# FlowEternal/multitask-hydranet

Measured on AMD Instinct MI355X. Metric: images/sec (fwd+bwd) HydraNet @ default res, 1/2/4/8 MI355X; CPU-ref same run, higher is better.
Workload: dtype bf16; 1 GPU; full HydraNet (backbone + BiFPN + seg/det/lane heads + multitask loss), big cfg, fwd+loss+bwd; batch_per_gpu=16, global_batch=16, resolution=3x512x1024, parallelism=dp1, hipgraph=True

## Files before the change

include/hydranet_hip.h:

```cpp
#ifndef HYDRANET_HIP_H
#define HYDRANET_HIP_H

#ifdef __cplusplus
extern "C" {
#endif

typedef struct ihipStream_t* hipStream_t;


int hn_gconv_pack_diag(const float* w, void* wk, void* wd, int C, hipStream_t stream);
int hn_pack_weight(const float* w, void* wp, void* wt, int Cout, int Cin, int taps, hipStream_t stream);
int hn_pack_weight_ex(const float* w, void* wp, void* wt, int Cout, int Cin_total, int ci0, int Cin, int taps, int phase, const float* bias,
                      float* b_eff, hipStream_t stream);
int hn_phase_fold(const float* dw_eff, const float* dw1, const float* db_eff, float* dw, float* db, int K, int C0, int C1, hipStream_t stream);
int hn_pack_weights_batched(const long* jobs, int njobs, long total_blocks, const int* block_job, hipStream_t stream);
int hn_pack_small_batched(const long* jobs, const int* block_job, long total_blocks, hipStream_t stream);

int hn_conv_gemm_nt(const void* x0, const void* x1, int mode, int n_img, int H, int W, int C0, int C1, int ld0, int ld1, int up, long M,
                    const void* w, int Nout, int KP, int taps, const float* bias, int act, void* out, int out_f32, int ldc, long rpi,
                    long img_stride, float* psum, float* psq, hipStream_t stream);
int hn_nt_stat_rows(long M, int Nout);
int hn_nt_stat_tile(long M, int Nout);
int hn_direct_stat_rows(int n_img, int H, int W);
int hn_conv_gemm_nt_imgw(const void* x0, int ld0, long M, int C0, const void* w, long w_img_stride, long rows_per_image, int Nout, int KP,
                         const float* bias, int act, void* out, int ldc, const void* addend, int ld_add, hipStream_t stream);
int hn_scale_weight_gate(const void* wp, const float* gate, void* out, int N, int Cout, int C, int KP, hipStream_t stream);
int hn_conv_gemm_nt_lvl(const void* x0, int ld0, long M, int C0, const void* w, int Nout, int KP, const float* bias, int act, void* out,
                        int ldc, const float* coef, int nlev, const long* rows, hipStream_t stream);
int hn_conv_gemm_nt_lvlout(const void* x0, int ld0, long M, int C0, const void* w, int Nout, int KP, const float* bias, int act, float* out,
                           int ldc, long img_stride, int n_img, int nlev, const int* H, const int* W, int row_align, hipStream_t stream);

int hn_conv_gemm_nt_ex(const void* x0, const void* x1, int mode, int n_img, int H, int W, int C0, int C1, int ld0, int ld1, int up, long M,
                       const void* w, int Nout, int KP, int taps, const float* bias, int act, void* out, int out_f32, int ldc, long rpi,
                       long img_stride, float* psum, float* psq, const float* xscale, const float* xshift, const float* xgate, long xhw,
                       int xact, const void* addend, int ld_add, int add_mode, hipStream_t stream);
int hn_conv_gemm_nt_stat(const void* x0, const void* x1, int mode, int n_img, int H, int W, int C0, int C1, int ld0, int ld1, int up, long M,
                         const void* w, int Nout, int KP, int taps, const float* bias, int act, void* out, int out_f32, int ldc, long rpi,
                         long img_stride, float* psum, float* psq, const void* addend, int ld_add, int add_mode, int emode, const void* ez,
                         int ld_ez, const float* ecoef, hipStream_t stream);
int hn_conv_gemm_nt_stat3(const void* x0, int ld0, long M, int C0, const void* w, int Nout, int KP, void* out, int ldc, float* psum, float* psq,
                          const void* addend, int ld_add, const void* ez, int ld_ez, const void* ey, int ld_ey, const float* ecoef,
                          hipStream_t stream);
int hn_wgrad_plan(int mode, int n_img, int H, int W, long M, int Nout, int KP, int taps, int* splits, long* rows_per_split, long* ws_bytes);
int hn_conv_gemm_tn(const void* x0, const void* x1, int mode, int n_img, int H, int W, int C0, int C1, int ld0, int ld1, int up, long M,
                    const void* dz, int ldz, int Nout, int KP, int taps, float* workspace, float* dw, hipStream_t stream);


int hn_stem_fwd(const float* x, const float* w, void* z, void* patches, int N, int H, int W, hipStream_t stream);

int hn_gconv_pack(const float* w, void* wk, void* wd, int C, int flip, hipStream_t stream);
int hn_gconv_fwd(const void* in, int ldi, const void* wk, void* out, int ldo, int N, int Hi, int Wi, int C, int stride, hipStream_t stream);
int hn_gconv_dgrad_s2(const void* dz, int ldz, const void* wd, void* dx, int ldx, int N, int Hi, int Wi, int C, hipStream_t stream);
long hn_wgrad_chunks(long pixels, long items);
int hn_gconv_wgrad(const void* x, int ldx, const void* dz, int ldz, float* part, int N, int Hi, int Wi, int C, int stride,
                   hipStream_t stream);

int hn_dw_pack(const float* w, void* wk, void* wkf, int C, hipStream_t stream);
int hn_dwconv_fwd(const void* in, int ldi, const void* wk, void* out, int ldo, int N, int H, int W, int C, hipStream_t stream);
int hn_dwconv_fwd_levels(const void* in, int ldi, const void* wk, void* out, int ldo, int N, int C, int nlev, const int* H, const int* W,
                         int row_align, int accumulate, hipStream_t stream);
long hn_dwconv_wgrad_blocks(long strips, int C);
int hn_dwconv_wgrad(const void* x, int ldx, const void* dz, int ldz, float* part, int N, int H, int W, int C, hipStream_t stream);
int hn_dwconv_wgrad_levels(const void* x, int ldx, const void* dz, int ldz, float* part, int N, int C, int nlev, const int* H, const int* W,
                           int row_align, hipStream_t stream);
long hn_dwconv_bwd_blocks(long strips, int C);
long hn_dwconv_bwd_blocks_levels(int N, int C, int nlev, const int* H, const int* W);
int hn_dwconv_bwd_levels(const void* dz, int ldz, const void* x, int ldx, const void* wf, void* dx, int lddx, float* part, int N, int C,
                         int nlev, const int* H, const int* W, int row_align, int accumulate, hipStream_t stream);

int hn_maxpool_fwd(const void* in, int ldi, void* out, int ldo, int N, int H, int W, int C, int mode, hipStream_t stream);
int hn_maxpool_bwd(const void* in, int ldi, const void* dout, int ldd, void* dx, int ldx, const float* wscale, int N, int H, int W, int C,
                   int mode, hipStream_t stream);
int hn_maxpool_bwd2(const void* in, int ldi, const void* dout, int ldd, void* dx, int ldx, const float* wscale, void* arg_ws, int N, int H,
                    int W, int C, int mode, int accumulate, hipStream_t stream);

int hn_up2_fwd(const void* in, int ldi, void* out, int ldo, int N, int H, int W, int C, hipStream_t stream);
int hn_sum2x2(const void* g, int ldg, void* out, int ldo, const float* wscale, int N, int H, int W, int C, int accumulate, hipStream_t stream);

int hn_fuse_dweights(const float* pw, int blocks, const float* praw, int nw, float eps, float* dp, hipStream_t stream);
int hn_fuse_fwd(const void* const* in, const int* ld, const int* mode, const float* w, void* out, int ldo, int N, int H, int W, int C,
                hipStream_t stream);
int hn_fuse_fwd_raw(const void* const* in, const int* ld, const int* mode, const float* praw, int nw, float eps, float* wn, void* out, int ldo,
                    int N, int H, int W, int C, hipStream_t stream);
int hn_fuse_bwd_blocks(int N, int H, int W, int C);
int hn_fuse_bwd(const void* const* in, const int* ld, const int* mode, const float* w, const void* dout, int ldd, void* g, int ldg,
                void* const* din, const int* ldin, const int* acc, float* pw, int N, int H, int W, int C, hipStream_t stream);
int hn_fuse_bwd_arg(const void* const* in, const int* ld, const int* mode, const float* w, const void* dout, int ldd, void* g, int ldg,
                    void* const* din, const int* ldin, const int* acc, float* pw, void* const* arg_out, int N, int H, int W, int C,
                    hipStream_t stream);
int hn_maxpool_bwd_from_arg(const void* arg, const void* dout, int ldd, void* dx, int ldx, const float* wscale, int N, int H, int W, int C,
                            int mode, int accumulate, hipStream_t stream);

// ... 206 lines not shown
```

multitask_hydranet_amd/csrc/hn_gemm.hip:

```cpp
#include "hn_common.h"
#include <climits>

#ifdef HN_TUNING
#define HN_DBG(p) ((p).dbg)
#else
#define HN_DBG(p) 0
#endif

struct XSrc {
    const bf16* x0;
    const bf16* x1;
    int mode;
    int H, W;
    int Hi, Wi;
    int C0, C1;
    int ld0, ld1;
    int up;
    long M;
    int clamp;
    int diag;
};

__device__ __forceinline__ int border_idx(int v, int L, int clamp) {
    if (clamp == 2) return (v < 0 || v >= L) ? -1 : v;
// ... 60 lines not shown
    if (s.mode == 2) {
        int iy = oy + ky - 1, ix = ox + kx - 1;
        iy = iy < 0 ? -iy : (iy >= s.Hi ? 2 * s.Hi - 2 - iy : iy);
        ix = ix < 0 ? -ix : (ix >= s.Wi ? 2 * s.Wi - 2 - ix : ix);
        if (which) return s.C1 ? (((long)n * s.Hi + iy) * s.Wi + ix) * s.ld1 : -1;
        const int hh = s.Hi >> s.up, ww = s.Wi >> s.up;
        return (((long)n * hh + (iy >> s.up)) * ww + (ix >> s.up)) * s.ld0;
    }
    const int iy = oy - ky, ix = ox - kx;
    if (which || iy < 0 || iy >= s.Hi || ix < 0 || ix >= s.Wi) return -1;
    return (((long)n * s.Hi + iy) * s.Wi + ix) * s.ld0;
}

__device__ __forceinline__ void glds16(const bf16* src, char* lds_wave_base) {
    __builtin_amdgcn_global_load_lds((const __attribute__((address_space(1))) void*)src,
                                     (__attribute__((address_space(3))) void*)lds_wave_base, 16, 0, 0);
}

__device__ __forceinline__ int swz(int row, int piece) { return row * 128 + ((piece ^ (row & 7)) << 4); }
__device__ __forceinline__ int pswz32(int row) { return (row >> 1) & 2; }

struct GemmNT {
    XSrc x;
    const bf16* w;
    int Nout, KP, taps;
    const float* bias;
    int act;
    void* out;
    int ldc;
    float* psum;
    float* psq;
    long rpi;
    long img_stride;
    int d2s;
    const float* xscale; const float* xshift; const float* xgate; long xhw; int xact;
    const bf16* addend; int ld_add;
    int phase_mode, phase_span;
    int add_s2;
    long* amax;
    int add_pre;
    long w_img_stride; unsigned w_rpi;
    const float* lcoef; int ln; long lrow[HN_MAX_LEVELS + 1];
    int lo_n; unsigned lo_hw[HN_MAX_LEVELS]; unsigned lo_pix[HN_MAX_LEVELS];
    int fold;
    bf16* fold_out2; int ld_fo2;
    bf16* ring;
    const bf16* fold_y; int ld_fy;
    int emode; const bf16* ez; int ld_ez; const float* ecoef;
    const bf16* ey; int ld_ey;
    int tile_major;
    int wpre;
    unsigned long long* dbg_buf;
    int dbg;
};

struct StatCoef { f32x4 sc, sh, mu, rs; };
__device__ __forceinline__ StatCoef stat_coef(const float* ecoef, int Nout, int emode, int co0, bool ev) {
    StatCoef c;
    c.sc = c.sh = c.mu = c.rs = (f32x4){0.f, 0.f, 0.f, 0.f};
    if (ev) {
        c.sc = *reinterpret_cast<const f32x4*>(ecoef + co0);
        c.sh = *reinterpret_cast<const f32x4*>(ecoef + Nout + co0);
        if (emode == 2) {
            c.mu = *reinterpret_cast<const f32x4*>(ecoef + 2 * Nout + co0);
            c.rs = *reinterpret_cast<const f32x4*>(ecoef + 3 * Nout + co0);
        }
    }
    return c;
}
__device__ __forceinline__ void stat_terms4(int emode, const f32x4 q, const f32x4 z, const StatCoef& cf, float& a0, float& a1, float& a2, float& a3,
                                            float& b0, float& b1, float& b2, float& b3) {
    float t1[4], t2[4];
#pragma unroll
    for (int r = 0; r < 4; ++r) {
        const float pre = cf.sc[r] * z[r] + cf.sh[r];
        const float b = bfround(pre > 0.f ? pre : 0.f);
        const float g = pre > 0.f ? q[r] : 0.f;
        t1[r] = emode == 0 ? q[r] : (emode == 1 ? q[r] * b : g);
        t2[r] = emode == 0 ? q[r] * q[r] : g * (z[r] - cf.mu[r]) * cf.rs[r];
    }
    a0 += t1[0]; a1 += t1[1]; a2 += t1[2]; a3 += t1[3];
    b0 += t2[0]; b1 += t2[1]; b2 += t2[2]; b3 += t2[3];
}

template <int BC, int BP, int WGC, int WGP, bool OUT_F32, int R, bool XF = false, int KG = 1, bool PLAIN = false, bool EPRE = false>
__global__ __launch_bounds__(256 * KG) void gemm_nt_kernel(const GemmNT p) {
    static_assert(!XF || R == 2, "the register-staged operand transform is written for the double buffer");
    static_assert(!PLAIN || !XF, "the plain-rows form has no operand transform");
    static_assert(KG == 1 || (!XF && R == 2), "the K-group form is written for the plain double buffer");
    constexpr int WC = BC / WGC, WP = BP / WGP, TC = WC / 16, TP = WP / 16;
    constexpr int XR = BP / 32, WR = (BC + 31) / 32;
    constexpr int STAGE = (BC + BP) * 128;
    extern __shared__ __attribute__((aligned(16))) char smem[];
    const int tid = threadIdx.x & 255, kg = __builtin_amdgcn_readfirstlane(threadIdx.x >> 8), lane = tid & 63, wave = __builtin_amdgcn_readfirstlane(tid >> 6);
    const int wc = wave / WGP, wp = wave % WGP;
    const int ncy = (p.Nout + BC - 1) / BC;
    const int lid = xcd_remap(blockIdx.x, gridDim.x);
    const int c_tile = lid % ncy, p_tile = lid / ncy;
    const int c_blk = c_tile * BC;
    const long p_blk = (long)p_tile * BP;
    const int r0 = tid >> 3, lp = (tid & 7) ^ (r0 & 7), half = lp >> 2, sub = (lp & 3) * 8;
    const int kc = p.KP >> 5, Q = p.taps * kc, S = (((Q + 1) >> 1) + KG - 1) / KG;
    const int Ktot = p.taps * p.KP;

    int xn[XR], xy[XR], xx[XR];
#pragma unroll
    for (int i = 0; i < XR; ++i) {
        if constexpr (PLAIN) { xn[i] = 0; xy[i] = 0; xx[i] = 0; }
        else decomp_row(p.x, p_blk + r0 + 32 * i, xn[i], xy[i], xx[i]);
    }

    int* ty0 = reinterpret_cast<int*>(smem + R * KG * STAGE);
    int* tx0 = ty0 + 3 * p.x.H;
    int* ty1 = tx0 + 3 * p.x.W;
    int* tx1 = ty1 + 3 * p.x.H;
    if (!PLAIN && p.x.mode >= 2) {
        for (int i = tid; i < 3 * p.x.H; i += 256) {
            const int k = i / p.x.H, o = i - k * p.x.H;
            if (p.x.mode == 2) {
                int v = o + k - 1;
                v = border_idx(v, p.x.Hi, p.x.clamp);
                ty0[i] = v >> p.x.up;
                if (p.x.C1) ty1[i] = v;
            } else {
                const int v = o - k;
                ty0[i] = (v < 0 || v >= p.x.Hi) ? -1 : v;
            }
        }
        for (int i = tid; i < 3 * p.x.W; i += 256) {
            const int k = i / p.x.W, o = i - k * p.x.W;
            if (p.x.mode == 2) {
                int v = o + k - 1;
                v = border_idx(v, p.x.Wi, p.x.clamp);
                tx0[i] = v >> p.x.up;
                if (p.x.C1) tx1[i] = v;
            } else {
                const int v = o - k;
                tx0[i] = (v < 0 || v >= p.x.Wi) ? -1 : v;
            }
// ... 68 lines not shown
                if (pre_stat && ev && pix < p.x.M) pez[i][j] = *reinterpret_cast<const bf16x4*>(p.ez + pix * p.ld_ez + co0);
            }
        }
    }
    const bool pre_add = staged_ && p.addend && !p.add_pre, pre_e3 = staged_ && p.psum != nullptr && p.emode == 3;
    bf16x8 padd[PRE ? PRE : 1], pey[PRE ? PRE : 1], pzz[PRE ? PRE : 1];
    bool phas[PRE ? PRE : 1];
#pragma unroll
    for (int u = 0; u < PRE; ++u) {
        const int idx = tid + 256 * u, row = idx / NPC_, pc = idx % NPC_;
        const long pix = p_blk + row;
        const int co = c_blk + pc * 8;
        const bool ok = kg == 0 && idx < BP * NPC_ && pix < p.x.M && co < p.Nout;
        padd[u] = pey[u] = pzz[u] = zero8();
        phas[u] = false;
        if (ok && pre_add) {
            long arow = pix;
            bool has = true;
            if (p.add_s2) {
                const unsigned W = (unsigned)p.x.W, H = (unsigned)p.x.H;
                const unsigned x = (unsigned)pix % W, t = (unsigned)pix / W;
                const unsigned y = t % H, n = t / H;
                has = !((x | y) & 1u);
                arow = ((long)n * (H >> 1) + (y >> 1)) * (W >> 1) + (x >> 1);
            }
            phas[u] = has;
            if (has) padd[u] = ld8(p.addend + arow * p.ld_add + co);
        }
        if (ok && pre_e3) { pey[u] = ld8(p.ey + pix * p.ld_ey + co); pzz[u] = ld8(p.ez + pix * p.ld_ez + co); }
    }

    f32x4 acc[TC][TP];
#pragma unroll
    for (int i = 0; i < TC; ++i)
#pragma unroll
        for (int j = 0; j < TP; ++j) acc[i][j] = (f32x4){0.f, 0.f, 0.f, 0.f};

    constexpr int G = XR + WR;
    static_assert(R == 2 || BC >= 32, "deeper rings need every wave to issue the same number of loads");
    bf16x8 xraw[XF ? XR : 1];
    bool xval[XF ? XR : 1];
    int xch = 0;
    float* xcoef = reinterpret_cast<float*>(smem + R * KG * STAGE);
    if (XF) {
        const long img = p.xgate ? p_blk / p.xhw : 0;
        for (int i = tid; i < p.KP; i += 256) {
            const bool v = i < Ctot;
            xcoef[i] = v ? p.xscale[i] : 0.f;
            xcoef[p.KP + i] = v ? p.xshift[i] : 0.f;
            xcoef[2 * p.KP + i] = (v && p.xgate) ? p.xgate[img * Ctot + i] : 1.f;
        }
        __syncthreads();
    }
    for (int it = 0; it < S + R - 1; ++it) {
        if (it >= R - 1) {
            const int newer = (it < S ? it : S) - 1 - (it - (R - 1));
            if (XF) asm volatile("s_waitcnt vmcnt(0) lgkmcnt(0)\n\ts_barrier" ::: "memory");
            else if (R >= 4 && newer >= 2) asm volatile("s_waitcnt vmcnt(%0)\n\ts_barrier" ::"n"(2 * G) : "memory");
            else if (R >= 3 && newer >= 1) asm volatile("s_waitcnt vmcnt(%0)\n\ts_barrier" ::"n"(G) : "memory");
            else asm volatile("s_waitcnt vmcnt(0)\n\ts_barrier" ::: "memory");
        }
        bool xcv = false;
        if (it < S) {
            char* sW = smem + ((it % R) * KG + kg) * STAGE;
            char* sX = sW + BC * 128;
            const int q = 2 * (it * KG + kg) + half;
            const bool qv = q < Q;
            const int c = cidx * 32 + sub;
            const bool from0 = c < p.x.C0;
            const bool cv = qv && c < Ctot;
            const bf16* xbase = from0 ? p.x.x0 + c : p.x.x1 + (c - p.x.C0);
            const long ldx = from0 ? p.x.ld0 : p.x.ld1;
            if (XF) {
                xcv = cv;
                xch = c;
#pragma unroll
                for (int i = 0; i < XR; ++i) {
                    const int pix = from0 ? pix0[i] : pix1[i];
                    xval[i] = cv && pix >= 0;
                    const bf16* src = xval[i] ? xbase + (long)pix * ldx : g_zero_piece;
                    xraw[i] = ld8(src);
                }
            } else if constexpr (PLAIN) {
#pragma unroll
                for (int i = 0; i < XR; ++i) {
                    const bf16* src = (cv && xoff[i] >= 0) ? p.x.x0 + xoff[i] + c : g_zero_piece;
                    glds16(src, sX + (wave * 8 + 32 * i) * 128);
                }
            } else {
#pragma unroll
            for (int i = 0; i < XR; ++i) {
                const int pix = from0 ? pix0[i] : pix1[i];
                const bf16* src = (cv && pix >= 0) ? xbase + (long)pix * ldx : g_zero_piece;
                glds16(src, sX + (wave * 8 + 32 * i) * 128);
            }
            }
#pragma unroll
            for (int i = 0; i < WR; ++i) {
                if (wave * 8 + 32 * i < BC) {
                    const bf16* src = (qv && wo[i] >= 0) ? wimg + wo[i] + q * 32 : g_zero_piece;
                    glds16(src, sW + (wave * 8 + 32 * i) * 128);
                }
            }
            if constexpr (PLAIN) {
                cidx += 2 * KG;
            } else if (qv) {
                cidx += 2 * KG;
                if (cidx >= kc) {
                    while (cidx >= kc) { cidx -= kc; ++tap; }
                    if (tap < p.taps) retap();
                }
            }
        }
        if (it >= R - 1) {
            const char* sW = smem + (((it - (R - 1)) % R) * KG + kg) * STAGE;
            const char* sX = sW + BC * 128;
#pragma unroll
            for (int ks = 0; ks < 2; ++ks) {
                bf16x8 a[TC], b[TP];
                const int piece = ks * 4 + (lane >> 4);
#pragma unroll
                for (int i = 0; i < TC; ++i) a[i] = *reinterpret_cast<const bf16x8*>(sW + swz(wc * WC + i * 16 + (lane & 15), piece));
#pragma unroll
                for (int j = 0; j < TP; ++j) b[j] = *reinterpret_cast<const bf16x8*>(sX + swz(wp * WP + j * 16 + (lane & 15), piece));
#pragma unroll
                for (int i = 0; i < TC; ++i)
// ... 2711 lines not shown
        pix += p.lo_hw[l];
    }
    HN_CHECK_ARG(p.lrow[nlev] == M);
    return run_gemm_nt(p, 0, true, st);
}

__global__ __launch_bounds__(256) void scale_weight_gate_kernel(const bf16* wp, const float* gate, bf16* out, int N, int Cout, int C, int KP) {
    const unsigned k8n = (unsigned)KP >> 3;
    const unsigned total = (unsigned)N * (unsigned)Cout * k8n;
    for (unsigned idx = blockIdx.x * 256u + threadIdx.x; idx < total; idx += gridDim.x * 256u) {
        const unsigned t = idx / k8n, k8 = idx - t * k8n;
        const unsigned n = t / (unsigned)Cout, co = t - n * (unsigned)Cout;
        const bf16x8 v = ld8(wp + (long)co * KP + k8 * 8);
        bf16x8 o;
#pragma unroll
        for (int j = 0; j < 8; ++j) {
            const int k = (int)k8 * 8 + j;
            o[j] = f2bf(k < C ? bf2f(v[j]) * gate[(long)n * C + k] : 0.f);
        }
        st8(out + ((long)n * Cout + co) * KP + k8 * 8, o);
    }
}
extern "C" int hn_scale_weight_gate(const void* wp, const float* gate, void* out, int N, int Cout, int C, int KP, hipStream_t st) {
    HN_CHECK_ARG(wp && gate && out && N > 0 && Cout > 0 && C > 0 && C <= KP && (KP & 31) == 0 && (long)N * Cout * (KP >> 3) < (1L << 31));
    long b = ((long)N * Cout * (KP >> 3) + 255) / 256;
    if (b > 4096) b = 4096;
    hipLaunchKernelGGL(scale_weight_gate_kernel, dim3((unsigned)b), dim3(256), 0, st, (const bf16*)wp, gate, (bf16*)out, N, Cout, C, KP);
    HN_LAUNCH_CHECK();
}

extern "C" int hn_conv_gemm_nt_ex(const void* x0, const void* x1, int mode, int n_img, int H, int W, int C0, int C1, int ld0, int ld1,
                                  int up, long M, const void* w, int Nout, int KP, int taps, const float* bias, int act, void* out,
                                  int out_f32, int ldc, long rpi, long img_stride, float* psum, float* psq, const float* xscale,
                                  const float* xshift, const float* xgate, long xhw, int xact, const void* addend, int ld_add,
                                  int add_mode, hipStream_t st) {
    GemmNT p = nt_conv(x0, x1, mode, H, W, C0, C1, ld0, ld1, up, M, w, Nout, KP, taps, bias, act, out, ldc, rpi, img_stride, psum, psq);
    p.xscale = xscale; p.xshift = xshift; p.xgate = xgate; p.xhw = xhw; p.xact = xact;
    nt_addend(p, addend, ld_add, add_mode);
    return run_gemm_nt(p, n_img, out_f32, st);
}

extern "C" int hn_conv_gemm_nt_stat(const void* x0, const void* x1, int mode, int n_img, int H, int W, int C0, int C1, int ld0, int ld1,
                                    int up, long M, const void* w, int Nout, int KP, int taps, const float* bias, int act, void* out,
                                    int out_f32, int ldc, long rpi, long img_stride, float* psum, float* psq, const void* addend, int ld_add,
                                    int add_mode, int emode, const void* ez, int ld_ez, const float* ecoef, hipStream_t st) {
    HN_CHECK_ARG((emode == 1 || emode == 2) && psum && (psq || emode == 1) && ez && ecoef && (Nout & 7) == 0 && (ld_ez & 3) == 0 && !out_f32 &&
                 act == HN_ACT_NONE && (mode <= 1 || mode == 5) && (reinterpret_cast<uintptr_t>(ez) & 7) == 0);
    GemmNT p = nt_conv(x0, x1, mode, H, W, C0, C1, ld0, ld1, up, M, w, Nout, KP, taps, bias, act, out, ldc, rpi, img_stride, psum, psq);
    nt_addend(p, addend, ld_add, add_mode);
    p.emode = emode; p.ez = (const bf16*)ez; p.ld_ez = ld_ez; p.ecoef = ecoef;
    return run_gemm_nt(p, n_img, out_f32, st);
}

extern "C" int hn_conv_gemm_nt_stat3(const void* x0, int ld0, long M, int C0, const void* w, int Nout, int KP, void* out, int ldc, float* psum,
                                     float* psq, const void* addend, int ld_add, const void* ez, int ld_ez, const void* ey, int ld_ey,
                                     const float* ecoef, hipStream_t st) {
    HN_CHECK_ARG(psum && psq && ez && ey && ecoef && addend && (ld_ez & 7) == 0 && (ld_ey & 7) == 0);
    GemmNT p = nt_rows(x0, ld0, M, C0, w, Nout, KP, nullptr, HN_ACT_NONE, out, ldc);
    p.psum = psum; p.psq = psq;
    p.addend = (const bf16*)addend; p.ld_add = ld_add;
    p.emode = 3; p.ez = (const bf16*)ez; p.ld_ez = ld_ez; p.ecoef = ecoef; p.ey = (const bf16*)ey; p.ld_ey = ld_ey;
    return run_gemm_nt(p, 0, false, st);
}

extern "C" int hn_conv3x3_out_argmax(const void* x0, int n_img, int H, int W, int C0, int ld0, const void* w, int k, int KP, const float* bias,
                                     long* mask, hipStream_t st) {
    HN_CHECK_ARG(mask && k >= 1 && 4 * k <= 32 && 32 * 32 * k * 4 <= 32768 && KP == 64 && C0 <= 64 && ((2 * W * k) & 3) == 0 && ((32 * k) & 3) == 0 &&
                 (reinterpret_cast<uintptr_t>(mask) & 15) == 0);
    GemmNT p = nt_desc(make_xsrc(x0, nullptr, 4, H, W, C0, 0, ld0, 0, 0, (long)n_img * H * W), w, 4 * k, KP, 9, bias, HN_ACT_NONE, mask, 4 * k);
    p.d2s = k;
    p.amax = mask;
    return run_gemm_nt(p, n_img, true, st);
}

extern "C" int hn_conv3x3_phase(const void* x0, int mode, int n_img, int H, int W, int C0, int ld0, const void* w, int Nout, int KP,
                                const float* bias, int act, void* out, int ldc, int k, const void* addend, int ld_add, hipStream_t st) {
    HN_CHECK_ARG((mode == 4 || mode == 3) && k > 0 && (k & 3) == 0);
    if (mode == 4) HN_CHECK_ARG(Nout == 4 * k && (k % 64 == 0) && (!addend || (ld_add > 0 && (ld_add & 3) == 0)));
    else HN_CHECK_ARG(C0 == 4 * k && (k % 64 == 0) && !addend);
    GemmNT p = nt_desc(make_xsrc(x0, nullptr, mode, H, W, C0, 0, ld0, 0, 0, (long)n_img * H * W), w, Nout, KP, 9, bias, act, out, ldc);
    p.phase_mode = mode == 4 ? 1 : 2; p.phase_span = k;
    if (mode == 4) {
        p.d2s = k;
        if (addend) { p.addend = (const bf16*)addend; p.ld_add = ld_add; p.add_pre = 1; }
    }
    return run_gemm_nt(p, n_img, false, st);
}

__global__ __launch_bounds__(256) void seg_ring_fix_kernel(bf16* out, int ldo, const bf16* ring, const bf16* y, int ldy, int N, int H, int W,
                                                           int C, int clamp, int s2d, bf16* out2, int ld2) {
    const int C8 = C >> 3, T = 2 * W + 2 * (H - 2), R = 2 * (W + 2) + 2 * H;
    const long total = (long)N * T * C8;
    const long idx = (long)blockIdx.x * 256 + threadIdx.x;
    if (idx >= total) return;
    const int cg = (int)(idx % C8);
    long t = idx / C8;
    const int tt = (int)(t % T);
    const int n = (int)(t / T);
    const int ry0 = clamp ? 0 : 1, ry1 = clamp ? H - 1 : H - 2, rx0 = clamp ? 0 : 1, rx1 = clamp ? W - 1 : W - 2;
    int yy, xx;
    if (tt < W) { yy = ry0; xx = tt; }
    else if (tt < 2 * W) { yy = ry1; xx = tt - W; }
    else {
        int j = tt - 2 * W;
        xx = rx0;
        if (j >= H - 2) { j -= H - 2; xx = rx1; }
// ... 540 lines not shown
```

multitask_hydranet_amd/model.py:

```python
from __future__ import annotations

import contextlib
import itertools
import math
import sys
import weakref
from typing import Dict, List, Optional, Sequence

import numpy as np
import torch
import torch.nn as nn

from . import ops as K
from .ops import ACT_ELU, ACT_NONE, ACT_RELU, ACT_SIGMOID, ACT_SWISH

BN_STD = dict(eps=1e-5, momentum=0.1)
BN_FPN = dict(eps=1e-3, momentum=0.01)


def regnet_stages(initial_width, slope, quantized_param, network_depth, bottleneck_ratio, group_width):
    u = initial_width + slope * np.arange(network_depth)
    s = np.round(np.log(u / initial_width) / np.log(quantized_param))
    q = 8 * np.round(initial_width * np.power(quantized_param, s) / 8)
    widths, depths = np.unique(q.astype(np.int32), return_counts=True)
# ... 381 lines not shown

    def _backbone_shared(self, x, ext, tail=None):
        p = "backbone.net."
        x = x.contiguous().float()
        t = self._cba(x, p + "stem.conv", p + "stem.bn", BN_STD, kind="stem", act=ACT_RELU)
        feats = []
        P = self._idx
        for k, d in enumerate(self.depths):
            group = None
            names = [f"{p}stage_{k}.blocks.block_{i}.{c}" for i in range(d)
                     for c in ("conv_block_1.0.weight", "conv_block_2.0.weight", "conv_block_3.0.weight", "shortcut.0.weight", "se.1.weight",
                               "se.1.bias", "se.3.weight", "se.3.bias")]
            names = [nm for nm in names if nm in P]
            if (K.DEFER_WGRAD and self.training and torch.is_grad_enabled() and t.requires_grad and t.is_cuda and (self.se_ratio is not None) and
                    all(P[nm].requires_grad for nm in names)):
                group = K.WgradGroup()
                t = K.DeferredGrads.apply(t, group, *[P[nm] for nm in names])
            i = 0
            while i < d:
                q = f"{p}stage_{k}.blocks.block_{i}."
                if i > 0 and self.training and not (torch.is_grad_enabled() and t.requires_grad) and self._xstage_shape_ok(q, t):
                    while i < d:
                        j1 = min(d, i + 16)
                        params = []
                        for j in range(i, j1):
                            params += self._xblock_params(f"{p}stage_{k}.blocks.block_{j}.")
                        with torch.no_grad():
                            t = K.xstage_forward_raw(t, params, BN_STD["eps"], BN_STD["momentum"])["out"][j1 - i - 1]
                        i = j1
                    break
                if i > 0 and i < d and self._xstage_run(q, t, group):
                    while i < d:
                        j1 = min(d, i + 16)
                        params = []
                        for j in range(i, j1):
                            params += self._xblock_params(f"{p}stage_{k}.blocks.block_{j}.")
                        t = K.xstage_apply(t, group, BN_STD["eps"], BN_STD["momentum"], params)
                        i = j1
                    break
                t = self._xblock(q, t, self.backbone_stride if i == 0 else 1, group)
                i += 1
            last = k == len(self.depths) - 1
            if last and tail is not None and K.DEFER_WGRAD and self.training and torch.is_grad_enabled() and t.requires_grad and t.is_cuda:
                t = K.DeferredGrads.apply(t, tail[0], *tail[1])
                tail[2] = True
            al, slot = K.share(t, ext[k] + (0 if last else 1))
            feats.append((al[:ext[k]], slot))
            if not last:
                t = al[-1]
        return feats

    def _sepconv(self, name, x, act=ACT_NONE):
        P = self._idx
        d = K.DwConv.apply(x, P[name + ".depthwise_conv.conv.weight"])
        return self._cba(d, name + ".pointwise_conv.conv", name + ".bn", BN_FPN, act=act)

    def _fusew(self, name):
        return self._idx[name]

    CELL_IN_COUNTS = (1, 2, 2, 2, 2)

    def _cell_shared(self, p, inputs, first, ext):
        red = lambda nm, src, i: self._cba(src[0][i], p + nm + ".0.conv", p + nm + ".1", BN_FPN, act=ACT_NONE, slot=src[1])
        sh = K.share
        if first:
            if len(inputs) == 4:
                p3, p4, p5 = inputs[-3:]
                p6_in = K.MaxPool.apply(red("p5_to_p6", p5, 2), 0)
            else:
                p3, p4, p5, p6r = inputs[-4:]
                p6_in = red("p6_down_channel", p6r, 0)
            (p6a, p6b, p6c), s6 = sh(p6_in, 3)
            p7_in = K.MaxPool.apply(p6c, 0)
            p3a, s3 = red("p3_down_channel", p3, 0), None
            (p4a, p4b), s4a, s4b = (red("p4_down_channel", p4, 0), red("p4_down_channel_2", p4, 1)), None, None
            (p5a, p5b), s5a, s5b = (red("p5_down_channel", p5, 0), red("p5_down_channel_2", p5, 1)), None, None
        else:
            (p3a,), s3 = inputs[0]
            (p4a, p4b), s4a = inputs[1]
            (p5a, p5b), s5a = inputs[2]
            (p6a, p6b), s6 = inputs[3]
            s4b, s5b = s4a, s5a
        if first:
            (p7a, p7b), s7 = sh(p7_in, 2)
        else:
            (p7a, p7b), s7 = inputs[4]
        F = K.Fuse.apply
        w = lambda nm: self._fusew(p + nm)
        (u6a, u6b), t6 = sh(self._sepconv(p + "conv6_up", F(w("p6_w1"), 1, 2, 0, p6a, p7a, None, (s6, s7, None))), 2)
        (u5a, u5b), t5 = sh(self._sepconv(p + "conv5_up", F(w("p5_w1"), 1, 2, 0, p5a, u6a, None, (s5a, t6, None))), 2)
        (u4a, u4b), t4 = sh(self._sepconv(p + "conv4_up", F(w("p4_w1"), 1, 2, 0, p4a, u5a, None, (s4a, t5, None))), 2)
        o3, q3 = sh(self._sepconv(p + "conv3_up", F(w("p3_w1"), 1, 2, 0, p3a, u4a, None, (s3, t4, None))), 1 + ext[0])
        o4, q4 = sh(self._sepconv(p + "conv4_down", F(w("p4_w2"), 1, 1, 3, p4b, u4b, o3[0], (s4b, t4, q3))), 1 + ext[1])
        o5, q5 = sh(self._sepconv(p + "conv5_down", F(w("p5_w2"), 1, 1, 3, p5b, u5b, o4[0], (s5b, t5, q4))), 1 + ext[2])
        o6, q6 = sh(self._sepconv(p + "conv6_down", F(w("p6_w2"), 1, 1, 3, p6b, u6b, o5[0], (s6, t6, q5))), 1 + ext[3])
        o7, q7 = sh(self._sepconv(p + "conv7_down", F(w("p7_w2"), 1, 3, 0, p7b, o6[0], None, (s7, q6, None))), ext[4])
        return [(o3[1:], q3), (o4[1:], q4), (o5[1:], q5), (o6[1:], q6), (o7, q7)]

    def first_cell_counts(self):
        n = len(self.depths)
        cnt = [0] * n
        if n == 4:
            cnt[-3:] = [1, 2, 3]
        else:
            cnt[-4:] = [1, 2, 2, 1]
        return cnt

    def _cell(self, p, inputs, first):
# ... 326 lines not shown
```

multitask_hydranet_amd/ops/neck.py:

```python
from __future__ import annotations

import ctypes
import os
from typing import Optional, Sequence, Tuple

import torch

from .._lib import lib, policy
from .core import *
from .backbone import *


def k_dwconv(x, wk, out=None):
    n, h, w, c = x.shape
    if out is None:
        out = new_act(n, h, w, c, x.device)
    lib().call("hn_dwconv_fwd", ptr(x), ld(x), ptr(wk), ptr(out), ld(out), n, h, w, c)
    return out


def k_dwconv_wgrad(x, dz):
    n, h, w, c = x.shape
    chunks = lib().query("hn_dwconv_wgrad_blocks", n * h * ((w + 3) // 4), c)
    part = torch.empty((chunks, c * 9), device=x.device, dtype=F32)
    lib().call("hn_dwconv_wgrad", ptr(x), ld(x), ptr(dz), ld(dz), ptr(part), n, h, w, c)
    return k_rows_reduce(part, 1, chunks, c * 9).view(c, 1, 3, 3)


def k_dwconv_bwd(dz, x, wf, geom=None, want_dx=True, into=None, queue=None, weight=None):
    c = x.shape[3]
    if geom is None:
        n, h, w, _ = x.shape
        H, W, nl, align = (ctypes.c_int * 1)(h), (ctypes.c_int * 1)(w), 1, 1
    else:
        nl, H, W, _, _ = _geom_arrays(geom)
        n, align = geom[0], LEVEL_ALIGN
    blocks = lib().query("hn_dwconv_bwd_blocks_levels", n, c, nl, ctypes.addressof(H), ctypes.addressof(W))
    part = torch.empty((blocks, c * 9), device=x.device, dtype=F32)
    dx = None
    if want_dx:
        dx = torch.empty_like(dz) if into is None else into
    lib().call("hn_dwconv_bwd_levels", ptr(dz), ld(dz), ptr(x), ld(x), ptr(wf), ptr(dx), ld(dx) if dx is not None else 0, ptr(part), n, c, nl,
               ctypes.addressof(H), ctypes.addressof(W), align, 0 if into is None else 1)
    if queue is not None:
        queue.add_rows(weight, part, blocks, c * 9, (c, 1, 3, 3))
        return dx, None
    return dx, k_rows_reduce(part, 1, blocks, c * 9).view(c, 1, 3, 3)


class DwConv(torch.autograd.Function):
    @staticmethod
    def forward(ctx, x, weight):
        wk, wf = pack_dw_weight(weight)
        ctx.queue, ctx.wref = (cur_queue() if weight.requires_grad else None), weight
        ctx.save_for_backward(x, wf)
        return k_dwconv(x, wk)

    @staticmethod
    def backward(ctx, dout):
        x, wf = ctx.saved_tensors
        dout = dense(dout)
        return k_dwconv_bwd(dout, x, wf, want_dx=ctx.needs_input_grad[0], queue=ctx.queue, weight=ctx.wref)


def k_maxpool(x, mode, out=None):
    n, h, w, c = x.shape
    if out is None:
        out = new_act(n, h // 2, w // 2, c, x.device)
    lib().call("hn_maxpool_fwd", ptr(x), ld(x), ptr(out), ld(out), n, h, w, c, mode)
    return out


def k_maxpool_bwd(x, dout, mode, wscale=None, into=None, accumulate=False):
    n, h, w, c = x.shape
    dx = new_act(n, h, w, c, x.device) if into is None else into
    arg = torch.empty((n * (h // 2) * (w // 2) * c,), device=x.device, dtype=torch.uint8)
    lib().call("hn_maxpool_bwd2", ptr(x), ld(x), ptr(dout), ld(dout), ptr(dx), ld(dx), ptr(wscale), ptr(arg), n, h, w, c, mode,
               1 if accumulate else 0)
    return dx


class MaxPool(torch.autograd.Function):
    @staticmethod
    def forward(ctx, x, mode):
        ctx.mode = mode
        ctx.save_for_backward(x)
        return k_maxpool(x, mode)

    @staticmethod
    def backward(ctx, dout):
        (x,) = ctx.saved_tensors
        return k_maxpool_bwd(x, dense(dout), ctx.mode), None


def _fuse_args(ins, modes):
    arr_p = (ctypes.c_void_p * 3)(*[ptr(t) if t is not None else None for t in ins])
    arr_l = (ctypes.c_int * 3)(*[ld(t) if t is not None else 0 for t in ins])
    arr_m = (ctypes.c_int * 3)(*modes)
    return arr_p, arr_l, arr_m


class GradSlot:
    __slots__ = ("buf",)

    def __init__(self):
        self.buf = None


class Share(torch.autograd.Function):

    @staticmethod
    def forward(ctx, x, slot, n):
        ctx.slot = slot
        ctx.set_materialize_grads(False)
        return tuple(x.view_as(x) for _ in range(n))
# ... 101 lines not shown
```

Before: 982.2 images/sec.

## Fuse depthwise 3x3 conv into pointwise GEMM prologue for BiFPN sepconvs

Adds a DW template variant of the NT GEMM kernel. It computes the 3x3 depthwise convolution on the fly from the input while staging the A operand, writes the depthwise output once for backward, and feeds it straight into the pointwise GEMM with BN statistics. In training, a new autograd function routes BiFPN separable convs through this kernel, so the separate depthwise kernel launch and one re-read of its output are gone. The cost is nine neighbour loads per row inside the GEMM loop and a full waitcnt barrier each iteration, which may lower MFMA overlap.

```diff
diff --git a/include/hydranet_hip.h b/include/hydranet_hip.h
--- a/include/hydranet_hip.h
+++ b/include/hydranet_hip.h
@@ -38,6 +38,8 @@
                          const void* w, int Nout, int KP, int taps, const float* bias, int act, void* out, int out_f32, int ldc, long rpi,
                          long img_stride, float* psum, float* psq, const void* addend, int ld_add, int add_mode, int emode, const void* ez,
                          int ld_ez, const float* ecoef, hipStream_t stream);
+int hn_sepconv_fwd(const void* x, int ldx, int n_img, int H, int W, int C, const void* dwk, void* d, int ldd, const void* w, int Nout, int KP,
+                   const float* bias, int act, void* out, int ldc, float* psum, float* psq, hipStream_t stream);
 int hn_conv_gemm_nt_stat3(const void* x0, int ld0, long M, int C0, const void* w, int Nout, int KP, void* out, int ldc, float* psum, float* psq,
                           const void* addend, int ld_add, const void* ez, int ld_ez, const void* ey, int ld_ey, const float* ecoef,
                           hipStream_t stream);
diff --git a/multitask_hydranet_amd/csrc/hn_gemm.hip b/multitask_hydranet_amd/csrc/hn_gemm.hip
--- a/multitask_hydranet_amd/csrc/hn_gemm.hip
+++ b/multitask_hydranet_amd/csrc/hn_gemm.hip
@@ -136,6 +136,7 @@
     int wpre;
     unsigned long long* dbg_buf;
     int dbg;
+    const bf16* dwk; bf16* dwout; int ld_dwout;
 };
 
 struct StatCoef { f32x4 sc, sh, mu, rs; };
@@ -167,8 +168,10 @@
     b0 += t2[0]; b1 += t2[1]; b2 += t2[2]; b3 += t2[3];
 }
 
-template <int BC, int BP, int WGC, int WGP, bool OUT_F32, int R, bool XF = false, int KG = 1, bool PLAIN = false, bool EPRE = false>
+template <int BC, int BP, int WGC, int WGP, bool OUT_F32, int R, bool XF = false, int KG = 1, bool PLAIN = false, bool EPRE = false,
+          bool DW = false>
 __global__ __launch_bounds__(256 * KG) void gemm_nt_kernel(const GemmNT p) {
+    static_assert(!DW || (R == 2 && KG == 1 && !XF && !PLAIN && !EPRE && !OUT_F32), "the depthwise prologue is a plain double-buffer form");
     static_assert(!XF || R == 2, "the register-staged operand transform is written for the double buffer");
     static_assert(!PLAIN || !XF, "the plain-rows form has no operand transform");
     static_assert(KG == 1 || (!XF && R == 2), "the K-group form is written for the plain double buffer");
@@ -343,10 +346,18 @@
         }
         __syncthreads();
     }
+    bf16* dwl = reinterpret_cast<bf16*>(smem + R * KG * STAGE);
+    if constexpr (DW) {
+        for (int i = tid; i < 9 * p.KP; i += 256) {
+            const int tp = i / p.KP, ch = i - tp * p.KP;
+            dwl[i] = ch < p.x.C0 ? p.dwk[tp * p.x.C0 + ch] : (bf16)0.0f;
+        }
+        __syncthreads();
+    }
     for (int it = 0; it < S + R - 1; ++it) {
         if (it >= R - 1) {
             const int newer = (it < S ? it : S) - 1 - (it - (R - 1));
-            if (XF) asm volatile("s_waitcnt vmcnt(0) lgkmcnt(0)\n\ts_barrier" ::: "memory");
+            if (XF || DW) asm volatile("s_waitcnt vmcnt(0) lgkmcnt(0)\n\ts_barrier" ::: "memory");
             else if (R >= 4 && newer >= 2) asm volatile("s_waitcnt vmcnt(%0)\n\ts_barrier" ::"n"(2 * G) : "memory");
             else if (R >= 3 && newer >= 1) asm volatile("s_waitcnt vmcnt(%0)\n\ts_barrier" ::"n"(G) : "memory");
             else asm volatile("s_waitcnt vmcnt(0)\n\ts_barrier" ::: "memory");
@@ -362,7 +373,45 @@
             const bool cv = qv && c < Ctot;
             const bf16* xbase = from0 ? p.x.x0 + c : p.x.x1 + (c - p.x.C0);
             const long ldx = from0 ? p.x.ld0 : p.x.ld1;
-            if (XF) {
+            if constexpr (DW) {
+#pragma unroll 1
+                for (int i = 0; i < XR; ++i) {
+                    const long m = p_blk + r0 + 32 * i;
+                    const long t = m / p.x.W;
+                    const int ox = (int)(m - t * p.x.W), oy = (int)(t % p.x.H);
+                    const bool rv = cv && m < p.x.M;
+                    bf16x8 win[9];
+#pragma unroll
+                    for (int ky = 0; ky < 3; ++ky)
+#pragma unroll
+                        for (int kx = 0; kx < 3; ++kx) {
+                            const int iy = oy + ky - 1, ix = ox + kx - 1;
+                            const bool ok = rv && iy >= 0 && iy < p.x.H && ix >= 0 && ix < p.x.W;
+                            win[ky * 3 + kx] = ld8(ok ? p.x.x0 + (m + (long)(ky - 1) * p.x.W + (kx - 1)) * p.x.ld0 + c : g_zero_piece);
+                        }
+                    bf16x8 o = zero8();
+                    if (rv) {
+                        float a[8];
+#pragma unroll
+                        for (int k = 0; k < 8; ++k) a[k] = 0.f;
+#pragma unroll
+                        for (int ky = 0; ky < 3; ++ky) {
+                            const int iy = oy + ky - 1;
+                            if (iy < 0 || iy >= p.x.H) continue;
+#pragma unroll
+                            for (int kx = 0; kx < 3; ++kx) {
+                                const bf16x8 w8 = *reinterpret_cast<const bf16x8*>(dwl + (ky * 3 + kx) * p.KP + c);
+#pragma unroll
+                                for (int k = 0; k < 8; ++k) a[k] = fmaf(bf2f(win[ky * 3 + kx][k]), bf2f(w8[k]), a[k]);
+                            }
+                        }
+#pragma unroll
+                        for (int k = 0; k < 8; ++k) o[k] = f2bf(a[k]);
+                        if (c_tile == 0 && c < p.x.C0) st8(p.dwout + m * p.ld_dwout + c, o);
+                    }
+                    *reinterpret_cast<bf16x8*>(sX + (wave * 8 + 32 * i) * 128 + lane * 16) = o;
+                }
+            } else if (XF) {
                 xcv = cv;
                 xch = c;
 #pragma unroll
@@ -3180,6 +3229,36 @@
     return run_gemm_nt(p, n_img, out_f32, st);
 }
 
+template <int BC, int BP, int WGC, int WGP>
+static int launch_nt_dw(const GemmNT& p, hipStream_t st) {
+    dim3 grid(cdiv(p.x.M, BP) * cdiv(p.Nout, BC));
+    const size_t lds = (size_t)(BC + BP) * 128 * 2 + (size_t)9 * p.KP * sizeof(bf16);
+    static std::atomic<unsigned long long> optin{0};
+    if (lds > 64 * 1024 && !lds_optin(optin, {(const void*)gemm_nt_kernel<BC, BP, WGC, WGP, false, 2, false, 1, false, false, true>}))
+        return HN_ERR_LAUNCH;
+    hipLaunchKernelGGL((gemm_nt_kernel<BC, BP, WGC, WGP, false, 2, false, 1, false, false, true>), grid, dim3(256), lds, st, p);
+    HN_LAUNCH_CHECK();
+}
+
+extern "C" int hn_sepconv_fwd(const void* x, int ldx, int n_img, int H, int W, int C, const void* dwk, void* d, int ldd, const void* w, int Nout,
+                              int KP, const float* bias, int act, void* out, int ldc, float* psum, float* psq, hipStream_t st) {
+    const long M = (long)n_img * H * W;
+    HN_CHECK_ARG(x && dwk && d && w && out && n_img > 0 && H > 0 && W > 0 && M < (1L << 31) && C > 0 && (C & 7) == 0 && C <= KP &&
+                 (KP & 31) == 0 && ((ldx | ldd) & 7) == 0 && ldx >= C && ldd >= C && aligned16(x) && aligned16(d) && Nout > 0 &&
+                 Nout <= 128 && ldc >= Nout && (psum || !psq));
+    GemmNT p = nt_rows(x, ldx, M, C, w, Nout, KP, bias, act, out, ldc);
+    p.x.H = H; p.x.W = W;
+    p.psum = psum; p.psq = psq;
+    p.dwk = (const bf16*)dwk; p.dwout = (bf16*)d; p.ld_dwout = ldd;
+    if (small_tile(M, Nout)) return launch_nt_dw<128, 64, 2, 2>(p, st);
+    switch (pick_bc(Nout)) {
+        case 16: return launch_nt_dw<16, 128, 1, 4>(p, st);
+        case 32: return launch_nt_dw<32, 128, 1, 4>(p, st);
+        case 64: return launch_nt_dw<64, 128, 2, 2>(p, st);
+        default: return launch_nt_dw<128, 128, 2, 2>(p, st);
+    }
+}
+
 extern "C" int hn_conv_gemm_nt_stat3(const void* x0, int ld0, long M, int C0, const void* w, int Nout, int KP, void* out, int ldc, float* psum,
                                      float* psq, const void* addend, int ld_add, const void* ez, int ld_ez, const void* ey, int ld_ey,
                                      const float* ecoef, hipStream_t st) {
diff --git a/multitask_hydranet_amd/model.py b/multitask_hydranet_amd/model.py
--- a/multitask_hydranet_amd/model.py
+++ b/multitask_hydranet_amd/model.py
@@ -457,8 +457,12 @@
 
     def _sepconv(self, name, x, act=ACT_NONE):
         P = self._idx
+        pw = name + ".pointwise_conv.conv"
+        if self.training and K.sepconv_ok(x, P[pw + ".weight"]):
+            return K.sepconv_bn_act(x, P[name + ".depthwise_conv.conv.weight"], P[pw + ".weight"], P.get(pw + ".bias"), self._bn(name + ".bn"),
+                                    act=act, **BN_FPN)
         d = K.DwConv.apply(x, P[name + ".depthwise_conv.conv.weight"])
-        return self._cba(d, name + ".pointwise_conv.conv", name + ".bn", BN_FPN, act=act)
+        return self._cba(d, pw, name + ".bn", BN_FPN, act=act)
 
     def _fusew(self, name):
         return self._idx[name]
diff --git a/multitask_hydranet_amd/ops/neck.py b/multitask_hydranet_amd/ops/neck.py
--- a/multitask_hydranet_amd/ops/neck.py
+++ b/multitask_hydranet_amd/ops/neck.py
@@ -61,6 +61,72 @@
         x, wf = ctx.saved_tensors
         dout = dense(dout)
         return k_dwconv_bwd(dout, x, wf, want_dx=ctx.needs_input_grad[0], queue=ctx.queue, weight=ctx.wref)
+
+
+SEPCONV_FUSED = policy("HN_SEPCONV_FUSED", "1") != "0"
+
+
+def sepconv_ok(x, w_pw):
+    return SEPCONV_FUSED and FUSED_BN and x.dim() == 4 and x.dtype == BF16 and x.shape[3] % 8 == 0 and w_pw.shape[0] <= 128 and \
+        w_pw.shape[1] == x.shape[3]
+
+
+def k_sepconv(x, wk, wp, cout, bias=None, stats=True):
+    n, h, w, c = x.shape
+    d = new_act(n, h, w, c, x.device)
+    z = new_act(n, h, w, cout, x.device)
+    psum = psq = None
+    if stats:
+        pr = lib().query("hn_nt_stat_rows", n * h * w, cout)
+        psum = torch.empty((pr, cout), device=x.device, dtype=F32)
+        psq = torch.empty((pr, cout), device=x.device, dtype=F32)
+    lib().call("hn_sepconv_fwd", ptr(x), ld(x), n, h, w, c, ptr(wk), ptr(d), ld(d), ptr(wp), cout, kp32(c), ptr(bias), ACT_NONE, ptr(z), ld(z),
+               ptr(psum), ptr(psq))
+    return d, z, psum, psq
+
+
+class SepConvBnAct(torch.autograd.Function):
+
+    @staticmethod
+    def forward(ctx, x, w_dw, w_pw, conv_bias, gamma, beta, rm, rv, nbt, act, eps, momentum):
+        n, h, w, c = x.shape
+        cout = w_pw.shape[0]
+        wk, wf = pack_dw_weight(w_dw)
+        wp, wt = pack_conv_weight(w_pw)
+        d, z, psum, psq = k_sepconv(x, wk, wp, cout, bias=conv_bias)
+        count = n * h * w
+        out, coef, _, _ = k_bn_apply_fused(z, psum, psq, count, gamma, beta, eps, momentum, rm, rv, act, training=True)
+        if nbt is not None:
+            nbt.add_(1)
+        ctx.act, ctx.count, ctx.wt = act, count, wt
+        ctx.has_bias = conv_bias is not None
+        ctx.pw_queue = cur_queue() if w_pw.requires_grad else None
+        ctx.dw_queue = cur_queue() if w_dw.requires_grad else None
+        ctx.pw_ref, ctx.dw_ref = w_pw, w_dw
+        ctx.save_for_backward(x, wf, d, z, coef)
+        return out
+
+    @staticmethod
+    def backward(ctx, dout):
+        x, wf, d, z, coef = ctx.saved_tensors
+        dout = dense(dout)
+        n, h, w, cout = z.shape
+        cin = x.shape[3]
+        grid = (n, h, w)
+        dbias = torch.empty((cout,), device=z.device, dtype=F32) if ctx.has_bias else None
+        dz, dgamma, dbeta, _ = bn_backward_fused(dout, z, None, coef, ctx.act, ctx.count, zero_c=dbias)
+        dd, _, _ = k_gemm_nt(dz, None, 0, grid, ctx.wt, cin, kp32(cout), 1)
+        if ctx.pw_queue is not None:
+            dw_pw = ctx.pw_queue.add_gemm(ctx.pw_ref, d, dz, 0, grid, cin, cout)
+        else:
+            dw_pw = k_gemm_tn(d, None, 0, grid, dz, cout, kp32(cin), 1, cin)
+        dx, dw_dw = k_dwconv_bwd(dd, x, wf, want_dx=ctx.needs_input_grad[0], queue=ctx.dw_queue, weight=ctx.dw_ref)
+        return dx, dw_dw, dw_pw, dbias, dgamma, dbeta, None, None, None, None, None, None
+
+
+def sepconv_bn_act(x, w_dw, w_pw, conv_bias, bn, act=ACT_NONE, eps=1e-5, momentum=0.1):
+    gamma, beta, rm, rv, nbt = bn
+    return SepConvBnAct.apply(x, w_dw, w_pw, conv_bias, gamma, beta, rm, rv, nbt, act, eps, momentum)
 
 
 def k_maxpool(x, mode, out=None):
```

Result: slower. 972.0 images/sec (median of 2 runs) (-1.0%).
